# pwrliang/grpc-rdma

Hardware: AMD Instinct MI355X
Metric: streaming GiB/s @1 MiB msgs (client-streaming, 1 connection per GPU) (higher is better)
Workload: dtype u8

## Files before the change

grpc-rdma_amd/csrc/grdma_dev.h:

```cpp
#ifndef GRDMA_DEV_H
#define GRDMA_DEV_H

#include <stddef.h>
#include <stdint.h>

#define GRDMA_ALIGN 8ull
#define GRDMA_RESERVED 24ull
#define GRDMA_FOOTER 0xFFFFFFFFFFFFFFFFull

#define GRDMA_MAX_SEGS 16384
#define GRDMA_MAX_SLICES 8192
#define GRDMA_TX_MAX_RECORDS 4096
#define GRDMA_HINT_MAX_RECORDS 8192
#define GRDMA_RX_HIST 1024
#define GRDMA_RX_TAB_SLOTS 8u
#define GRDMA_RX_TAB_STRIDE 516u
#define GRDMA_RX_TAB_WORDS (4u + 6u * GRDMA_RX_TAB_STRIDE)
#define GRDMA_RX_TAB_MAGIC 0x7AB1E5u
#define GRDMA_RX_HIST_ALLOC_WORDS (GRDMA_RX_HIST + GRDMA_RX_TAB_SLOTS * GRDMA_RX_TAB_WORDS)
#define GRDMA_TILE_BYTES 8192ull
#define GRDMA_PLAN_TILE_SHIFT(ring_cap) ((ring_cap) >= (32ull << 20) ? 14u : 13u)
#define GRDMA_MIN_READ_SLICE 256ull

#ifndef GRDMA_PAIR_STATUS_DEFINED
// ... 127 lines not shown
  uint64_t consumed;
  uint64_t records;
  uint64_t would_block;
  uint64_t credit_sent;
  uint64_t credit_head;
  uint64_t head, moving_head, remain;
  uint64_t arena_used;
  uint64_t zero_off[2];
  uint64_t zero_len[2];
  uint64_t seq;
  uint64_t commit_seq;
  uint32_t pad1;
  uint32_t pad0;
  uint64_t dbg[16];
};

struct grdma_plan {
  uint32_t nsegs;
  uint32_t ntiles;
  uint64_t bytes;
  uint64_t tag_base;
  uint64_t tag_mask;
  uint32_t tile_bytes;
  uint32_t ready;
  struct grdma_seg segs[GRDMA_MAX_SEGS];
  uint32_t tile_prefix[GRDMA_MAX_SEGS + 1];
  uint32_t pad_line0[31];
  uint32_t blocks_done;
  uint32_t mw_arrive;
  uint32_t promise_done;
  uint32_t pad_p;
  uint64_t promise;
  uint32_t mw_done;
  uint32_t pad_line1[25];
};
static_assert(offsetof(grdma_plan, promise) % 8 == 0, "the hand-over word is a 64-bit atomic");

#define GRDMA_JOB_HOOK_ARGS 10
struct grdma_job_hook {
  const void* fn;
  uint32_t grid, threads;
  uint64_t args[GRDMA_JOB_HOOK_ARGS];
};

#endif
```

grpc-rdma_amd/csrc/grdma_rx_fast.h:

```cpp
#ifndef GRDMA_RX_FAST_H
#define GRDMA_RX_FAST_H
#include "grdma_dev.h"
#include "grdma_devfn.h"
#include "grdma_ops.h"

namespace {

#define RXF_THREADS 1024
#define RXF_PER 4
#define RXF_KERNEL_ATTR
#define RXF_MAX (RXF_THREADS * RXF_PER)
#define RXF_WAVES (RXF_THREADS / 64)
#define RXF_MINRD 256u
#define RXF_PMAX 512u
#define RXF_LOOKBACK 192u

__device__ unsigned long long g_rx_fast_drains[6] = {0, 0, 0, 0, 0, 0};

#define RXG_BULK 4096
#define RXG_PAD(i) ((i) + ((i) >> 4))
struct rx_lds_general {
  uint32_t hist[GRDMA_RX_HIST];
  uint32_t penc[RXG_PAD(RXG_BULK) + 1];
  uint32_t xenc[RXG_PAD(RXG_BULK + 1) + 1];
// ... 78 lines not shown
__device__ __forceinline__ rxf_layout rxf_lay(uint32_t n, uint32_t s_in, uint32_t pay, uint32_t cap, uint32_t cap_open,
                                              bool odd, uint32_t ts) {
  rxf_layout L;
  const rxf_rec rp = rxf_replay(n, s_in);
  L.sl0 = (rp.sl0 == RXF_MINRD && s_in != 0) ? cap_open : rp.sl0;
  L.sl1 = rp.sl1;
  L.sl_cnt = rp.sl_cnt;
  L.bytes = rxf_al16(L.sl0) + rxf_al16(L.sl1);
  const uint32_t filled = s_in ? cap_open - s_in : 0;
  const uint32_t d2 = (odd && rp.c2) ? rxf_al16(cap_open) : filled + rp.c1;
  const uint32_t mask = cap - 1;
  const uint32_t p0 = pay, l_a = rp.c1 < cap - p0 ? rp.c1 : cap - p0;
  const uint32_t p2 = (pay + rp.c1) & mask, l_c = rp.c2 < cap - p2 ? rp.c2 : cap - p2;
  L.off[0] = p0;  L.len[0] = l_a;          L.dst_rel[0] = filled;
  L.off[1] = 0;   L.len[1] = rp.c1 - l_a;  L.dst_rel[1] = filled + l_a;
  L.off[2] = p2;  L.len[2] = l_c;          L.dst_rel[2] = d2;
  L.off[3] = 0;   L.len[3] = rp.c2 - l_c;  L.dst_rel[3] = d2 + l_c;
  if (pay + n <= cap && L.len[2] != 0 && d2 == filled + rp.c1) {
    L.len[0] += L.len[2];
    L.len[2] = 0;
  }
  L.nsg = 0;
  L.ntl = 0;
#pragma unroll
  for (int k = 0; k < 4; k++) {
    L.nsg += L.len[k] ? 1u : 0u;
    L.ntl += rxf_tiles(L.len[k], ts);
  }
  return L;
}

struct rxf_counters {
  uint64_t total_read, credit_msgs, rx_records, rx_rounds, seq;
  uint32_t h1;
  grdma_hostline* line;
};
__device__ __forceinline__ rxf_counters rxf_load_counters(const grdma_conn* c, const grdma_rx_result* res) {
  return {c->total_read, c->credit_msgs, c->rx_records, c->rx_rounds, res->seq, c->rx_h1, c->line};
}

template <class Tail>
__device__ __forceinline__ void rxf_commit(const grdma_rx_op& op, bool cursors, uint8_t* ring, uint64_t cap64, uint64_t head64, uint64_t mh0,
                                           uint64_t irs0, uint32_t Lr, uint32_t ts,
                                           uint32_t V, uint32_t tot_n, uint32_t tot_sl, uint32_t tot_sg, uint32_t tot_tl, uint32_t tot_by,
                                           uint32_t short_len, uint32_t leftover_final,
                                           uint64_t slice_idx0, uint64_t a_off0, uint64_t a_end, uint64_t hc, const Tail& tail,
                                           bool crossed, uint64_t base, uint64_t credit, uint64_t credit_head, const rxf_counters& o,
                                           uint64_t t_begin, uint64_t t_pattern, uint64_t t_probe, uint64_t t_state, uint64_t t_scan,
                                           uint64_t t_emit, uint32_t P, uint32_t nwg, uint64_t d_arrived, uint64_t d_loaded,
                                           uint64_t d_credit) {
  grdma_conn* const c = op.conn;
  grdma_plan* const plan = op.plan;
  grdma_rx_result* const res = op.result;
  grdma_slice_out* const out_slices = op.slices + slice_idx0;
  const uint32_t nsl_final = tot_sl + (short_len ? 1u : 0u);
  const uint64_t Ctot = Lr;
  const uint64_t irs = crossed ? Ctot - base : irs0 + Ctot;
  const uint64_t nh = (head64 + Lr) & (cap64 - 1);
  if (short_len) {
    out_slices[tot_sl].off = a_off0 + tot_by;
    out_slices[tot_sl].len = short_len;
  }
  plan->nsegs = tot_sg;
  plan->ntiles = tot_tl;
  plan->tile_bytes = 1u << ts;
  plan->tile_prefix[tot_sg] = tot_tl;
  plan->bytes = tot_n;
  plan->tag_base = (uint64_t)ring;
  plan->tag_mask = cap64 - 1;
  plan->blocks_done = 0;
  c->head = nh;
// ... 27 lines not shown
  res->consumed = Lr;
  res->records = V;
  res->would_block = 1;
  res->credit_sent = credit;
  res->head = nh;
  res->moving_head = nh;
  res->remain = 0;
  res->arena_used = a_end;
  res->zero_off[0] = res->zero_off[1] = res->zero_len[0] = res->zero_len[1] = 0;
  if (nh > mh0) {
    res->zero_off[0] = mh0;
    res->zero_len[0] = nh - mh0;
  } else {
    res->zero_off[0] = mh0;
    res->zero_len[0] = cap64 - mh0;
    res->zero_off[1] = 0;
    res->zero_len[1] = nh;
  }
  res->dbg[0] = t_begin;
  res->dbg[2] = t_pattern - t_begin;
  res->dbg[3] = t_probe - t_begin;
  res->dbg[4] = t_state - t_begin;
  res->dbg[5] = t_scan - t_begin;
  res->dbg[6] = t_emit - t_begin;
  res->dbg[7] = V;
  res->dbg[8] = P;
  res->dbg[9] = 0xFA57;
  if (nwg) {
    res->dbg[10] = nwg;
    res->dbg[11] = d_arrived;
    res->dbg[12] = d_loaded;
    res->dbg[13] = d_credit;
  }
  res->pad1++;
  res->dbg[1] = __builtin_amdgcn_s_memtime();
  atomicAdd(&g_rx_fast_drains[0], 1ull);
  __hip_atomic_store(&res->seq, op.seq_next ? op.seq_next : o.seq + 1, __ATOMIC_RELAXED, __HIP_MEMORY_SCOPE_SYSTEM);
}

__device__ __forceinline__ void rxf_scan3(uint32_t v0, uint32_t v1, uint32_t v2, uint32_t (*s_w)[RXF_WAVES],
                                          uint32_t* x0, uint32_t* x1, uint32_t* x2, uint32_t tot[3]) {
  const int lane = threadIdx.x & 63, wave = threadIdx.x >> 6;
  const uint32_t i0 = wave_incl_scan_u32(v0), i1 = wave_incl_scan_u32(v1), i2 = wave_incl_scan_u32(v2);
  if (lane == 63) {
    s_w[0][wave] = i0;
    s_w[1][wave] = i1;
    s_w[2][wave] = i2;
  }
  __syncthreads();
  uint32_t b0 = 0, b1 = 0, b2 = 0, t0 = 0, t1 = 0, t2 = 0;
#pragma unroll
  for (int w = 0; w < RXF_WAVES; w++) {
    const uint32_t a = s_w[0][w], b = s_w[1][w], c = s_w[2][w];
    if (w < wave) { b0 += a; b1 += b; b2 += c; }
    t0 += a; t1 += b; t2 += c;
  }
  __syncthreads();
  *x0 = b0 + i0 - v0;
  *x1 = b1 + i1 - v1;
  *x2 = b2 + i2 - v2;
  tot[0] = t0; tot[1] = t1; tot[2] = t2;
}

#define RXFP(i) ((i) + ((i) / RXF_PER))

__device__ __forceinline__ bool rxf_body(const grdma_rx_op& op_in) {
  const grdma_rx_op op = op_in;
// ... 327 lines not shown
```

grpc-rdma_amd/csrc/grdma_rx_hint.h:

```cpp
#ifndef GRDMA_RX_HINT_H
#define GRDMA_RX_HINT_H
#include <type_traits>
#include "grdma_rx_multi.h"

namespace {

#define RXH_HALF (RXM_G * RXM_THREADS)
#define RXH_MAX (2 * RXH_HALF)
static_assert(RXH_MAX <= GRDMA_HINT_MAX_RECORDS, "the size table of a round covers a drain");

struct rx_lds_hint {
  uint32_t n[RXH_MAX];
  uint32_t x[RXH_MAX + 1];
};

struct rxh_pre {
  uint32_t nv[RXH_HALF / RXM_THREADS];
  uint32_t V;
  uint64_t h_start;
};
__device__ __forceinline__ void rxh_preload(const grdma_rx_op& op, rxh_pre& p) {
  constexpr uint32_t PER = RXH_HALF / RXM_THREADS;
  const grdma_size_hint* const hint = op.sizes_in;
  p.V = 0;
  p.h_start = ~0ull;
#pragma unroll
  for (uint32_t r = 0; r < PER; r++) p.nv[r] = 0;
  if (hint != nullptr) {
    p.h_start = hint->start_off;
    p.V = hint->count;
#pragma unroll
    for (uint32_t r = 0; r < PER; r++) p.nv[r] = hint->n[threadIdx.x * PER + r];
  }
}

template <bool EWT = false, class RingWait = ring_ready_now, class Publish = credit_unpublished>
__device__ __forceinline__ int rxh_body(const grdma_rx_op& op_in, const uint32_t wg, const uint32_t nwg, const rxh_pre* pre = nullptr,
                                        RingWait* ring_wait = nullptr, Publish* publish = nullptr) {
  static_assert(sizeof(rx_lds_hint) <= sizeof(rx_lds), "the tables fit the planners' LDS");
  rx_lds_hint& H = *reinterpret_cast<rx_lds_hint*>(rx_lds_get());
  const grdma_rx_op op = op_in;
  const uint64_t t_begin = __builtin_amdgcn_s_memtime();
  const uint32_t tid = threadIdx.x;
  grdma_conn* c = op.conn;
  grdma_plan* plan = op.plan;
  grdma_rx_result* res = op.result;
  __shared__ uint32_t s_w[4][RXM_WAVES];
  __shared__ uint32_t s_bad, s_bad_ring, s_first, s_F;

  uint8_t* const ring = c->ring;
  const uint64_t cap64 = c->cap;
  const uint64_t head64 = c->head, mh0 = c->moving_head, remain0 = c->remain, leftover0 = c->leftover_cap;
  const uint64_t irs0 = c->internal_read_size;
  const uint64_t hc = c->rx_hist_count;
  const uint32_t status = c->status;
  const uint64_t lim = op.limit_ptr ? __hip_atomic_load(op.limit_ptr, __ATOMIC_RELAXED, __HIP_MEMORY_SCOPE_AGENT) : 0;
  const uint64_t slice_idx0 = op.append == 1 ? c->rx_slice_idx : 0;
  const uint64_t a_off0 = op.append == 1 ? c->rx_arena_off : 0;
  const grdma_size_hint* const hint = op.sizes_in;
  const uint64_t h_start = pre ? pre->h_start : (hint ? hint->start_off : ~0ull);
  const uint32_t V = pre ? pre->V : (hint ? hint->count : 0);

  const bool search_due = V > RXH_HALF && c->rx_period == 0 && hc >= c->rx_period_retry_at;
  bool ok = !search_due && status == GRDMA_PAIR_CONNECTED && op.raw_cap == 0 && op.append != 0 && !op.inline_apply &&
            op.limit_ptr != nullptr && remain0 == 0 && leftover0 <= RXF_MINRD && cap64 <= (1ull << 31) &&
            a_off0 < (1ull << 31) && hint != nullptr && h_start == head64 && V != 0 && V <= nwg * RXM_CHUNK && V <= RXH_MAX;
  uint64_t max_slices = GRDMA_MAX_SLICES;
  {
    const uint64_t room = op.slices_cap > slice_idx0 ? op.slices_cap - slice_idx0 : 0;
    if (room < max_slices) max_slices = room;
    if (op.max_reads < max_slices) max_slices = op.max_reads;
  }
  const uint32_t cap = (uint32_t)cap64, mask = cap - 1u, head = (uint32_t)head64;
  const uint32_t Lr = ((uint32_t)lim - head) & mask;
  const bool idle = Lr == 0;
  if (tid == 0) {
    s_bad = 0;
    s_bad_ring = 0;
    s_first = RXM_NONE;
    s_F = RXM_NONE;
  }
  __syncthreads();
  uint32_t reason = (!ok || idle) ? 1u : 0u;
  const uint32_t ts = GRDMA_PLAN_TILE_SHIFT(cap64);

  constexpr uint32_t PER = RXH_HALF / RXM_THREADS;
  if (!reason) {
    bool bad = false;
    uint32_t base_x = 0;
    auto load_half = [&](auto HALF) {
      constexpr uint32_t half = decltype(HALF)::value;
      uint32_t nv[PER];
      const uint32_t i0 = half * RXH_HALF + tid * PER;
#pragma unroll
      for (uint32_t r = 0; r < PER; r++)
        nv[r] = (half == 0 && pre) ? pre->nv[r] : hint->n[i0 + r < V ? i0 + r : 0];
      uint32_t sum = 0;
#pragma unroll
      for (uint32_t r = 0; r < PER; r++) {
        if (i0 + r >= V) nv[r] = 0;
        else bad |= nv[r] == 0 || nv[r] > cap - (uint32_t)GRDMA_RESERVED;
        sum += i0 + r < V ? 16u + ((nv[r] + 7u) & ~7u) : 0u;
      }
      uint32_t px, d1, d2, d3, tot[4];
      rxm_scan4(sum, 0, 0, 0, s_w, &px, &d1, &d2, &d3, tot);
      px += base_x;
#pragma unroll
      for (uint32_t r = 0; r < PER; r++) {
        H.n[i0 + r] = nv[r];
        H.x[i0 + r] = px;
        px += i0 + r < V ? 16u + ((nv[r] + 7u) & ~7u) : 0u;
      }
      if (tid == RXM_THREADS - 1) H.x[(half + 1) * RXH_HALF] = px;
      base_x += tot[0];
    };
    load_half(std::integral_constant<uint32_t, 0>{});
    if (V > RXH_HALF) load_half(std::integral_constant<uint32_t, 1>{});
    if (bad) s_bad = 1;
    __syncthreads();
    if (s_bad || H.x[V] != Lr) reason = 2;
  }
  const uint64_t t_pattern = __builtin_amdgcn_s_memtime();
  if (ring_wait != nullptr) (*ring_wait)();

  const uint32_t i_mine = wg * RXM_CHUNK + tid;
  const bool have = !reason && i_mine < V;
  uint32_t xe = 0, n_mine = 0;
  if (!reason) {
    typedef uint32_t u32x2 __attribute__((ext_vector_type(2)));
    const uint32_t ring_lo = (uint32_t)__builtin_amdgcn_readfirstlane((int)(uint32_t)(uint64_t)ring);
    const uint32_t ring_hi = (uint32_t)__builtin_amdgcn_readfirstlane((int)(uint32_t)((uint64_t)ring >> 32));
    const uint64_t ring_u = ((uint64_t)ring_hi << 32) | (uint64_t)ring_lo;
    const uint32_t cap_u = (uint32_t)__builtin_amdgcn_readfirstlane((int)cap);
    const __amdgpu_buffer_rsrc_t rs = __builtin_amdgcn_make_buffer_rsrc((void*)ring_u, 0, cap_u, 0x00020000);
    uint32_t ee = 0;
    if (have) {
      xe = H.x[i_mine];
      n_mine = H.n[i_mine];
      ee = 16u + ((n_mine + 7u) & ~7u);
    }
    const uint32_t o_h = have ? ((head + xe) & mask & ~7u) : 0u;
    const uint32_t o_f = have ? ((head + xe + ee - 8u) & mask & ~7u) : 0u;
    const u32x2 hw = __builtin_amdgcn_raw_buffer_load_b64(rs, o_h, 0, 16 );
    const u32x2 fw = __builtin_amdgcn_raw_buffer_load_b64(rs, o_f, 0, 16);
    if (have) {
      const uint64_t h = ((uint64_t)hw.y << 32) | hw.x, f = ((uint64_t)fw.y << 32) | fw.x;
      if (h != (uint64_t)n_mine || f != GRDMA_FOOTER) s_bad_ring = 1;
// ... 62 lines not shown
      m_by = Lm.bytes;
    }
    if (far) s_bad = 1;
    uint32_t d0, d1, d2, d3, ta[4], tz[4], tm[4];
    rxm_scan4(a_pk, a_tl, a_by, a_n, s_w, &d0, &d1, &d2, &d3, ta);
    rxm_scan4(z_pk, z_tl, z_by, z_n, s_w, &d0, &d1, &d2, &d3, tz);
    rxm_scan4(m_pk, m_tl, m_by, have ? n_mine : 0u, s_w, &x_pk, &x_tl, &x_by, &d3, tm);
    b_pk = ta[0]; b_tl = ta[1]; b_by = ta[2];
    tot_pk = ta[0] + tm[0] + tz[0];
    tot_tl = ta[1] + tm[1] + tz[1];
    tot_by = ta[2] + tm[2] + tz[2];
    tot_n = ta[3] + tm[3] + tz[3];
    if (s_bad) reason = 4;
    if (!reason) {
      bool far2 = false;
      s_end = rxf_space_after(H.n[V - 1], state_of(V - 1, &far2));
    }
  }
  const uint64_t t_state = __builtin_amdgcn_s_memtime();
  const uint32_t tot_sl = tot_pk & 0xFFFFu, tot_sg = tot_pk >> 16;
  const uint32_t cap_open_end = (odd_open && first_done == RXM_NONE) ? s0 : RXF_MINRD;
  const uint32_t short_len = s_end ? cap_open_end - s_end : 0;
  const uint32_t nsl_final = tot_sl + (short_len ? 1u : 0u);
  const uint32_t leftover_final = s_end ? s_end : RXF_MINRD;
  const uint64_t a_end = a_off0 + tot_by + rxf_al16(short_len);
  if (!reason && !(nsl_final + 2 <= max_slices && tot_sg + 8 <= GRDMA_MAX_SEGS && a_end + leftover_final + 16 <= op.arena_cap &&
                   a_end < (1ull << 32)))
    reason = 5;
  const uint64_t t_scan = __builtin_amdgcn_s_memtime();
  const bool committer = wg == nwg - 1;
  GRDMA_WAIT_LOADS();
  __syncthreads();
  if (tid == 0) drain_count_in(plan, reason);

  grdma_slice_out* const out_slices = op.slices + slice_idx0;
  if (!reason && have) {
    const uint32_t pk = b_pk + x_pk;
    uint32_t sl = pk & 0xFFFFu, sg = pk >> 16, tl = b_tl + x_tl;
    const uint64_t A = a_off0 + b_by + x_by;
    int last_piece = 0;
#pragma unroll
    for (int k = 1; k < 4; k++)
      if (Lm.len[k]) last_piece = k;
#pragma unroll
    for (int k = 0; k < 4; k++) {
      if (Lm.len[k] == 0) continue;
      const uint64_t fl = GRDMA_SEG_ZERO_SRC | (k == 0 ? GRDMA_SEG_TAG_HDR : 0) | (k == last_piece ? GRDMA_SEG_TAG_FTR : 0);
      xwg_put_seg<EWT>(&plan->segs[sg], (uint64_t)op.arena + A + Lm.dst_rel[k], (uint64_t)(ring + Lm.off[k]), (uint64_t)Lm.len[k], fl);
      xwg_st32<EWT>(&plan->tile_prefix[sg], tl);
      sg++;
      tl += rxf_tiles(Lm.len[k], ts);
    }
    uint64_t sof = A;
    if (Lm.sl0) {
      xwg_st64<EWT>(&out_slices[sl].off, sof);
      xwg_st64<EWT>(&out_slices[sl].len, (uint64_t)Lm.sl0);
      sl++;
      sof += rxf_al16(Lm.sl0);
    }
    if (Lm.sl1) {
      xwg_st64<EWT>(&out_slices[sl].off, sof);
      xwg_st64<EWT>(&out_slices[sl].len, (uint64_t)Lm.sl1);
    }
  }
  rxf_counters o = {};
  uint64_t base = 0, credit = 0, credit_head = 0;
  bool crossed = false;
  if (tid == 0 && !reason && committer) {
    o = rxf_load_counters(c, res);
    const uint64_t T = cap64 / 2, Ctot = Lr;
    uint64_t thr = T - irs0;
    while (Ctot >= thr) {
      uint32_t lo = 0, hi = V - 1;
      const uint32_t t32 = (uint32_t)thr;
      while (lo < hi) {
        const uint32_t mid = (lo + hi) >> 1;
        if (H.x[mid + 1] >= t32) hi = mid; else lo = mid + 1;
      }
      const uint32_t n = H.n[lo];
      bool far = false;
      rxf_credit_step(n, rxf_replay(n, state_of(lo, &far)), (uint64_t)H.x[lo + 1], head64, cap64, T, thr, base, credit, credit_head, crossed);
    }
  }
  const uint64_t t_emit = __builtin_amdgcn_s_memtime();

  if (!committer) {
    if (EWT) GRDMA_WAIT_VMEM();
    __syncthreads();
    if (tid == 0) drain_leave(plan);
    return 0;
  }
  const uint32_t s_any = drain_verdicts(plan, nwg);
  if (s_any) {
    if (tid == 0) {
      atomicAdd(&g_rx_fast_drains[reason ? reason : 3u], 1ull);
      atomicAdd(&g_rx_verdicts[s_any < nwg ? 0 : 1], 1ull);
      if (!idle) res->pad0++;
    }
    if (EWT) GRDMA_WAIT_VMEM();
    if (tid == 0) drain_close(plan, nwg);
    __syncthreads();
    return 2;
  }
  if (tid == 0 && publish != nullptr) (*publish)(credit, credit_head);

  constexpr int NH = GRDMA_RX_HIST / RXM_THREADS;
#pragma unroll
  for (int r = 0; r < NH; r++) {
    const uint32_t back = tid + r * RXM_THREADS;
    if (back < V) {
      const uint32_t i = V - 1 - back;
      c->rx_hist[(uint32_t)((hc + i) % GRDMA_RX_HIST)] = 16u + ((H.n[i] + 7u) & ~7u);
    }
  }
  if (tid == 0) {
    auto tail = [&](uint32_t& h1, uint32_t& h2) {
      h1 = 16u + ((H.n[V - 1] + 7u) & ~7u);
      h2 = V >= 2 ? 16u + ((H.n[V - 2] + 7u) & ~7u) : o.h1;
    };
    rxf_commit(op, true , ring, cap64, head64, mh0, irs0, Lr, ts,
               V, tot_n, tot_sl, tot_sg, tot_tl, tot_by, short_len, leftover_final,
               slice_idx0, a_off0, a_end, hc, tail,
               crossed, base, credit, credit_head, o,
               t_begin, t_pattern, t_probe, t_state, t_scan, t_emit, 0 , nwg, 0, 0, 0);
    drain_close(plan, nwg);
  }
  return 1;
}

}
#endif
```

grpc-rdma_amd/csrc/grdma_rx_multi.h:

```cpp
#ifndef GRDMA_RX_MULTI_H
#define GRDMA_RX_MULTI_H
#include "grdma_rx_fast.h"

namespace {

#define RXM_THREADS 256u
#define RXM_WAVES (RXM_THREADS / 64u)
#define RXM_G 16u
#define RXM_CHUNK RXM_THREADS
#define RXM_PFX (RXF_LOOKBACK + 1u)
#define RXM_RESET (2u * RXF_MINRD)
#define RXM_NONE 0xFFFFFFFFu

__device__ unsigned long long g_rx_tab_stats[2] = {0, 0};
__device__ unsigned long long g_rx_verdicts[2] = {0, 0};

struct rx_lds_multi {
  uint32_t hist[GRDMA_RX_HIST];
  uint32_t pat[RXF_PMAX], pre[RXF_PMAX + 1];
  uint32_t npat[RXF_PMAX];
  uint16_t sss[RXF_PMAX];
  uint32_t qpk[RXF_PMAX + 1], qtl[RXF_PMAX + 1], qby[RXF_PMAX + 1];
  uint32_t qn[RXF_PMAX + 1];
  uint16_t as[RXM_PFX + 1];
  uint32_t apk[RXM_PFX + 1], atl[RXM_PFX + 1], aby[RXM_PFX + 1];
};

__device__ __forceinline__ void rxm_scan4(uint32_t v0, uint32_t v1, uint32_t v2, uint32_t v3, uint32_t (*s_w)[RXM_WAVES],
                                          uint32_t* x0, uint32_t* x1, uint32_t* x2, uint32_t* x3, uint32_t tot[4]) {
  const int lane = threadIdx.x & 63, wave = threadIdx.x >> 6;
  const uint32_t i0 = wave_incl_scan_u32(v0), i1 = wave_incl_scan_u32(v1), i2 = wave_incl_scan_u32(v2), i3 = wave_incl_scan_u32(v3);
  if (lane == 63) {
    s_w[0][wave] = i0;
    s_w[1][wave] = i1;
    s_w[2][wave] = i2;
    s_w[3][wave] = i3;
  }
  __syncthreads();
  uint32_t b0 = 0, b1 = 0, b2 = 0, b3 = 0, t0 = 0, t1 = 0, t2 = 0, t3 = 0;
#pragma unroll
  for (int w = 0; w < (int)RXM_WAVES; w++) {
    const uint32_t a = s_w[0][w], b = s_w[1][w], c = s_w[2][w], d = s_w[3][w];
    if (w < wave) { b0 += a; b1 += b; b2 += c; b3 += d; }
    t0 += a; t1 += b; t2 += c; t3 += d;
  }
  __syncthreads();
  *x0 = b0 + i0 - v0;
  *x1 = b1 + i1 - v1;
  *x2 = b2 + i2 - v2;
  *x3 = b3 + i3 - v3;
  tot[0] = t0; tot[1] = t1; tot[2] = t2; tot[3] = t3;
}

__device__ __forceinline__ uint32_t rxm_div(uint32_t k, uint32_t P, uint32_t inv) { return P > 1 ? (uint32_t)(((uint64_t)k * inv) >> 32) : k; }

__device__ __forceinline__ void rxm_cyc(const rx_lds_multi& M, uint32_t P, uint32_t inv, uint32_t k, uint32_t* pk, uint32_t* tl, uint32_t* by) {
  const uint32_t q = rxm_div(k, P, inv), r = k - q * P;
  *pk = q * M.qpk[P] + M.qpk[r];
  *tl = q * M.qtl[P] + M.qtl[r];
  *by = q * M.qby[P] + M.qby[r];
}

__device__ unsigned long long g_wire_wait_runout = 0;
__device__ __forceinline__ void wire_arrive(grdma_plan* wp) {
  __builtin_amdgcn_fence(__ATOMIC_RELEASE, "agent");
  __hip_atomic_fetch_add(&wp->mw_arrive, 1u, __ATOMIC_RELAXED, __HIP_MEMORY_SCOPE_AGENT);
}
__device__ __forceinline__ void wire_wait(grdma_plan* wp, uint32_t wire_groups, uint32_t participants) {
  if (threadIdx.x == 0) {
    bool seen = false;
    for (uint32_t spins = 0; spins < (1u << 22) && !seen; spins++) {
      seen = __hip_atomic_load(&wp->mw_arrive, __ATOMIC_RELAXED, __HIP_MEMORY_SCOPE_AGENT) >= wire_groups;
      if (!seen) __builtin_amdgcn_s_sleep(2);
    }
    if (!seen) atomicAdd(&g_wire_wait_runout, 1ull);
    const uint32_t prev = __hip_atomic_fetch_add(&wp->promise_done, 1u, __ATOMIC_RELAXED, __HIP_MEMORY_SCOPE_AGENT);
    if (prev + 1 == participants) {
      __hip_atomic_store(&wp->promise_done, 0u, __ATOMIC_RELAXED, __HIP_MEMORY_SCOPE_AGENT);
      __hip_atomic_store(&wp->mw_arrive, 0u, __ATOMIC_RELAXED, __HIP_MEMORY_SCOPE_AGENT);
    }
  }
  __syncthreads();
}
struct ring_ready_now {
  __device__ __forceinline__ void operator()() {}
};
struct ring_behind_wire {
  grdma_plan* wp;
  uint32_t wire_groups, participants;
  bool done;
  __device__ __forceinline__ void operator()() {
    if (wp != nullptr && !done) wire_wait(wp, wire_groups, participants);
    done = true;
  }
};
struct credit_unpublished {
  __device__ __forceinline__ void operator()(uint64_t, uint64_t) {}
};
struct credit_promised {
  grdma_plan* plan;
  uint32_t participants;
  bool done;
  __device__ __forceinline__ void operator()(uint64_t credit_sent, uint64_t credit_head) {
    if (plan != nullptr && !done) (void)promise_keep(plan, participants, credit_sent, credit_head);
    done = true;
  }
};

__device__ __forceinline__ void drain_count_in(grdma_plan* plan, uint32_t reason) {
  __hip_atomic_fetch_add(&plan->mw_arrive, 1u + (reason ? 0x10000u : 0u), __ATOMIC_RELAXED, __HIP_MEMORY_SCOPE_AGENT);
}
__device__ __forceinline__ void drain_leave(grdma_plan* plan) {
  __hip_atomic_fetch_add(&plan->mw_done, 1u, __ATOMIC_RELAXED, __HIP_MEMORY_SCOPE_AGENT);
}
__device__ __forceinline__ uint32_t drain_verdicts(grdma_plan* plan, uint32_t nwg) {
  __shared__ uint32_t s_declined;
  if (threadIdx.x == 0) {
    uint32_t v = 0;
    for (uint32_t spins = 0; spins < (1u << 22); spins++) {
      v = __hip_atomic_load(&plan->mw_arrive, __ATOMIC_RELAXED, __HIP_MEMORY_SCOPE_AGENT);
      if ((v & 0xFFFFu) >= nwg) break;
      __builtin_amdgcn_s_sleep(1);
    }
    s_declined = (v & 0xFFFFu) >= nwg ? (v >> 16) : nwg;
  }
  __syncthreads();
  return s_declined;
}
__device__ __forceinline__ void drain_close(grdma_plan* plan, uint32_t nwg) {
  for (uint32_t spins = 0; spins < (1u << 22); spins++) {
    if (__hip_atomic_load(&plan->mw_done, __ATOMIC_RELAXED, __HIP_MEMORY_SCOPE_AGENT) >= nwg - 1) break;
    __builtin_amdgcn_s_sleep(1);
  }
  __hip_atomic_store(&plan->mw_done, 0u, __ATOMIC_RELAXED, __HIP_MEMORY_SCOPE_AGENT);
  __hip_atomic_store(&plan->mw_arrive, 0u, __ATOMIC_RELAXED, __HIP_MEMORY_SCOPE_AGENT);
}

template <bool EWT = false, class RingWait = ring_ready_now, class Publish = credit_unpublished>
__device__ __forceinline__ int rxm_body(const grdma_rx_op& op_in, const uint32_t wg, const uint32_t nwg, RingWait* ring_wait = nullptr,
                                        Publish* publish = nullptr) {
  static_assert(sizeof(rx_lds_multi) <= sizeof(rx_lds), "the tables fit their LDS");
  rx_lds_multi& M = *reinterpret_cast<rx_lds_multi*>(rx_lds_get());
  const grdma_rx_op op = op_in;
  const uint64_t t_begin = __builtin_amdgcn_s_memtime();
  const uint32_t tid = threadIdx.x;
  grdma_conn* c = op.conn;
  grdma_plan* plan = op.plan;
  grdma_rx_result* res = op.result;
  __shared__ uint32_t s_w[4][RXM_WAVES];
  __shared__ uint32_t s_bad, s_vj, s_first, s_F, s_miss, s_lb;

  uint8_t* const ring = c->ring;
  const uint64_t cap64 = c->cap;
  const uint64_t head64 = c->head, mh0 = c->moving_head, remain0 = c->remain, leftover0 = c->leftover_cap;
  const uint64_t irs0 = c->internal_read_size;
  const uint64_t hc = c->rx_hist_count;
  const uint32_t P = c->rx_period;
  const uint32_t status = c->status;
  const uint32_t* const gh = c->rx_hist;
  const bool limited = op.limit_ptr != nullptr || c->wire_limit != 0;
  const uint64_t lim = op.limit_ptr ? __hip_atomic_load(op.limit_ptr, __ATOMIC_RELAXED, __HIP_MEMORY_SCOPE_AGENT)
                                    : __hip_atomic_load(&c->wire_recv.wire_tail, __ATOMIC_RELAXED, __HIP_MEMORY_SCOPE_SYSTEM);
  const uint64_t slice_idx0 = op.append == 1 ? c->rx_slice_idx : 0;
  const uint64_t a_off0 = op.append == 1 ? c->rx_arena_off : 0;
  constexpr int NH = GRDMA_RX_HIST / RXM_THREADS;
  uint32_t hv[NH];
#pragma unroll
  for (int r = 0; r < NH; r++) hv[r] = gh[tid + r * RXM_THREADS];
// ... 3 lines not shown
            cap64 <= (1ull << 31) && a_off0 < (1ull << 31);
  uint64_t max_slices = GRDMA_MAX_SLICES;
  {
    const uint64_t room = op.slices_cap > slice_idx0 ? op.slices_cap - slice_idx0 : 0;
    if (room < max_slices) max_slices = room;
    if (op.max_reads < max_slices) max_slices = op.max_reads;
  }
  const uint32_t cap = (uint32_t)cap64, mask = cap - 1u, head = (uint32_t)head64;
  const uint32_t Lr = ((uint32_t)lim - head) & mask;
  const bool idle = Lr == 0;
  const uint32_t invP = P > 1 ? (uint32_t)(0xFFFFFFFFu / P) + 1u : 0u;
  auto divP = [&](uint32_t k) -> uint32_t { return rxm_div(k, P, invP); };
  if (tid == 0) {
    s_bad = 0;
    s_vj = RXM_NONE;
    s_first = RXM_NONE;
    s_F = RXM_NONE;
    s_miss = 0;
    s_lb = 0;
  }
  uint32_t c_hdr[4] = {0, 0, 0, 0}, c_key[2] = {0, 0}, c_sss[2] = {0, 0}, c_qpk[2] = {0, 0}, c_qtl[2] = {0, 0}, c_qby[2] = {0, 0},
           c_qn[2] = {0, 0}, c_tot[4] = {0, 0, 0, 0};
  uint32_t* c_tab = nullptr;
#pragma unroll
  for (int r = 0; r < NH; r++) M.hist[tid + r * RXM_THREADS] = hv[r];
  __syncthreads();
  uint32_t reason = (!ok || idle) ? 1u : 0u;

  uint32_t SP = 0, V = 0;
  if (!reason) {
    const uint32_t j0 = 2 * tid, j1 = j0 + 1;
    const uint32_t pv0 = j0 < P ? M.hist[(uint32_t)((hc - P + j0) % GRDMA_RX_HIST)] : 0;
    const uint32_t pv1 = j1 < P ? M.hist[(uint32_t)((hc - P + j1) % GRDMA_RX_HIST)] : 0;
    uint32_t px, d1, d2, d3, ptot[4];
    rxm_scan4(pv0 + pv1, 0, 0, 0, s_w, &px, &d1, &d2, &d3, ptot);
    SP = ptot[0];
    if (j0 < P) {
      M.pat[j0] = pv0;
      M.pre[j0] = px;
    }
    if (j1 < P) {
      M.pat[j1] = pv1;
      M.pre[j1] = px + pv0;
    }
    if (tid == 0) M.pre[P] = SP;
    const uint32_t q_full = SP ? Lr / SP : 0, rem = SP ? Lr - q_full * SP : 0;
    if (SP != 0) {
      if (j0 < P && px == rem) s_vj = j0;
      if (j1 < P && px + pv0 == rem) s_vj = j1;
    }
    __syncthreads();
    const uint32_t vj = s_vj;
    const uint64_t V64 = (uint64_t)q_full * P + vj;
    if (SP == 0 || vj == RXM_NONE || V64 == 0 || V64 > (uint64_t)nwg * RXM_CHUNK) reason = 2;
    else V = (uint32_t)V64;
  }
  const uint32_t ts = GRDMA_PLAN_TILE_SHIFT(cap64);
  const uint64_t t_pattern = __builtin_amdgcn_s_memtime();
  if (reason && !idle && op.sizes_in != nullptr) return 3;
  if (ring_wait != nullptr) (*ring_wait)();

  const uint32_t i_mine = wg * RXM_CHUNK + tid;
  const bool have = !reason && i_mine < V;
  const uint32_t PV = reason ? 0u : (V < P ? V : P);
  uint32_t xe = 0, ee = 0, ri_mine = 0, n_mine = 0;
  if (!reason) {
    typedef uint32_t u32x2 __attribute__((ext_vector_type(2)));
    const uint32_t ring_lo = (uint32_t)__builtin_amdgcn_readfirstlane((int)(uint32_t)(uint64_t)ring);
    const uint32_t ring_hi = (uint32_t)__builtin_amdgcn_readfirstlane((int)(uint32_t)((uint64_t)ring >> 32));
// ... 232 lines not shown
      while (hi - lo > 1) {
        const uint32_t mid = (lo + hi) >> 1;
        if (M.pre[mid] <= r) lo = mid; else hi = mid;
      }
      const uint32_t w = q * P + lo;
      if (w >= NF && w < V) {
        const uint32_t n = M.npat[lo], s = M.sss[lo];
        const rxf_layout La = rxf_lay(n, s, (head + q * SP + M.pre[lo] + 8u) & mask, cap, RXF_MINRD, false, ts);
        w_rec = w;
        d_sg = La.nsg - ((M.qpk[lo + 1] - M.qpk[lo]) >> 16);
        d_tl = La.ntl - (M.qtl[lo + 1] - M.qtl[lo]);
      }
    }
    if (V > NF) before(V, &tot_pk, &tot_tl, &tot_by);
    else { tot_pk = PS_pk; tot_tl = PS_tl; tot_by = PS_by; }
    uint32_t n_last;
    const uint32_t s_last_in = state_of(V - 1, &n_last);
    s_end = rxf_space_after(n_last, s_last_in);
  }
  const uint32_t tot_sl = tot_pk & 0xFFFFu, tot_sg = tot_pk >> 16;
  const uint32_t cap_open_end = (odd_open && first_done == RXM_NONE) ? s0 : RXF_MINRD;
  const uint32_t short_len = s_end ? cap_open_end - s_end : 0;
  const uint32_t nsl_final = tot_sl + (short_len ? 1u : 0u);
  const uint32_t leftover_final = s_end ? s_end : RXF_MINRD;
  const uint64_t a_end = a_off0 + tot_by + rxf_al16(short_len);
  if (!reason && !(nsl_final + 2 <= max_slices && tot_sg + 8 <= GRDMA_MAX_SEGS && a_end + leftover_final + 16 <= op.arena_cap &&
                   a_end < (1ull << 32)))
    reason = 5;
  const uint64_t t_scan = __builtin_amdgcn_s_memtime();
  const bool committer = wg == nwg - 1;
  GRDMA_WAIT_LOADS();
  __syncthreads();
  if (tid == 0) drain_count_in(plan, reason);

  grdma_slice_out* const out_slices = op.slices + slice_idx0;
  if (!reason && have) {
    uint32_t n, pk, tl, by;
    const uint32_t s_in = state_of(i_mine, &n);
    if (i_mine < NF) {
      pk = M.apk[i_mine];
      tl = M.atl[i_mine];
      by = M.aby[i_mine];
    } else {
      before(i_mine, &pk, &tl, &by);
    }
    uint32_t sl = pk & 0xFFFFu, sg = pk >> 16;
    const bool in_first = odd_open && i_mine <= first_done;
    const rxf_layout L = rxf_lay(n, s_in, (head + xe + 8u) & mask, cap, in_first ? s0 : RXF_MINRD,
                                 odd_open && i_mine == first_done, ts);
    const uint64_t A = a_off0 + by;
    int last_piece = 0;
#pragma unroll
    for (int k = 1; k < 4; k++)
      if (L.len[k]) last_piece = k;
#pragma unroll
    for (int k = 0; k < 4; k++) {
      if (L.len[k] == 0) continue;
      const uint64_t fl = GRDMA_SEG_ZERO_SRC | (k == 0 ? GRDMA_SEG_TAG_HDR : 0) | (k == last_piece ? GRDMA_SEG_TAG_FTR : 0);
      xwg_put_seg<EWT>(&plan->segs[sg], (uint64_t)op.arena + A + L.dst_rel[k], (uint64_t)(ring + L.off[k]), (uint64_t)L.len[k], fl);
      xwg_st32<EWT>(&plan->tile_prefix[sg], tl);
      sg++;
      tl += rxf_tiles(L.len[k], ts);
    }
    uint64_t sof = A;
    if (L.sl0) {
      xwg_st64<EWT>(&out_slices[sl].off, sof);
      xwg_st64<EWT>(&out_slices[sl].len, (uint64_t)L.sl0);
      sl++;
      sof += rxf_al16(L.sl0);
// ... 12 lines not shown
      const uint32_t qi = divP(i), ri = i - qi * P;
      return (uint64_t)qi * SP + M.pre[ri] + M.pat[ri];
    };
    const uint64_t T = cap64 / 2, Ctot = Lr;
    uint64_t thr = T - irs0;
    while (Ctot >= thr) {
      uint32_t lo;
      {
        const uint32_t t32 = (uint32_t)thr;
        const uint32_t qk = t32 / SP, r = t32 - qk * SP;
        uint32_t a = 0, b = P;
        if (r == 0) b = 0;
        while (b - a > 1) {
          const uint32_t mid = (a + b) >> 1;
          if (M.pre[mid] >= r) b = mid; else a = mid;
        }
        const uint32_t k = qk * P + b;
        lo = k ? k - 1 : 0;
        if (lo > V - 1) lo = V - 1;
      }
      uint32_t n;
      const uint32_t s_in = state_of(lo, &n);
      rxf_credit_step(n, rxf_replay(n, s_in), enc_end(lo), head64, cap64, T, thr, base, credit, credit_head, crossed);
    }
  }
  const uint64_t t_emit = __builtin_amdgcn_s_memtime();

  if (!committer) {
    if (EWT) GRDMA_WAIT_VMEM();
    __syncthreads();
    if (tid == 0) drain_leave(plan);
    return 0;
  }
  const uint32_t s_any = drain_verdicts(plan, nwg);
  if (c_fresh) {
    uint32_t* const a = c_tab + 4;
#pragma unroll
    for (int r = 0; r < 2; r++) {
      const uint32_t pj = 2 * tid + r;
      if (pj < P) {
        a[pj] = M.npat[pj];
        a[GRDMA_RX_TAB_STRIDE + pj] = (uint32_t)M.sss[pj];
        a[2 * GRDMA_RX_TAB_STRIDE + pj] = M.qpk[pj];
        a[3 * GRDMA_RX_TAB_STRIDE + pj] = M.qtl[pj];
        a[4 * GRDMA_RX_TAB_STRIDE + pj] = M.qby[pj];
        a[5 * GRDMA_RX_TAB_STRIDE + pj] = M.qn[pj];
      }
    }
    if (tid == 0) {
      a[2 * GRDMA_RX_TAB_STRIDE + RXF_PMAX] = M.qpk[P];
      a[3 * GRDMA_RX_TAB_STRIDE + RXF_PMAX] = M.qtl[P];
      a[4 * GRDMA_RX_TAB_STRIDE + RXF_PMAX] = M.qby[P];
      a[5 * GRDMA_RX_TAB_STRIDE + RXF_PMAX] = M.qn[P];
      c_tab[0] = P;
      c_tab[1] = ts;
      c_tab[2] = s_lb;
      c_tab[3] = GRDMA_RX_TAB_MAGIC;
    }
  }
  const uint64_t t_arrived = __builtin_amdgcn_s_memtime();
  if (s_any) {
    if (tid == 0) {
      atomicAdd(&g_rx_fast_drains[reason ? reason : 3u], 1ull);
      atomicAdd(&g_rx_verdicts[s_any < nwg ? 0 : 1], 1ull);
      if (!idle) res->pad0++;
    }
    if (EWT) GRDMA_WAIT_VMEM();
    if (tid == 0) drain_close(plan, nwg);
    __syncthreads();
    return 2;
  }
  if (tid == 0 && publish != nullptr) (*publish)(credit, credit_head);

  if (tid == 0) atomicAdd(&g_rx_tab_stats[c_hit ? 0 : 1], 1ull);
#pragma unroll
  for (int r = 0; r < NH; r++) {
    const uint32_t back = tid + r * RXM_THREADS;
    if (back < V) {
      const uint32_t i = V - 1 - back;
      c->rx_hist[(uint32_t)((hc + i) % GRDMA_RX_HIST)] = M.pat[i - divP(i) * P];
    }
  }
  if (tid == 0) {
    const uint64_t t_loaded = __builtin_amdgcn_s_memtime() + (o.seq & 0);
    const uint32_t tot_n = divP(V) * M.qn[P] + M.qn[V - divP(V) * P];
    const uint64_t t_credit = __builtin_amdgcn_s_memtime();
    auto tail = [&](uint32_t& h1, uint32_t& h2) {
      const uint32_t rl = (V - 1) - divP(V - 1) * P;
      h1 = M.pat[rl];
      h2 = V >= 2 ? M.pat[rl ? rl - 1 : P - 1] : o.h1;
    };
    rxf_commit(op, op.append != 0, ring, cap64, head64, mh0, irs0, Lr, ts,
               V, tot_n, tot_sl, tot_sg, tot_tl, tot_by, short_len, leftover_final,
               slice_idx0, a_off0, a_end, hc, tail,
               crossed, base, credit, credit_head, o,
               t_begin, t_pattern, t_probe, t_state, t_scan, t_emit, P, nwg, t_arrived - t_begin,
               t_loaded - t_begin, t_credit - t_begin);
    drain_close(plan, nwg);
  }
  return 1;
}

}
#endif
```

Measured before the change: 680.4.

## Use epoch-based drain counters and hoist history tail fetch before verdict wait

```diff
diff --git a/grpc-rdma_amd/csrc/grdma_dev.h b/grpc-rdma_amd/csrc/grdma_dev.h
--- a/grpc-rdma_amd/csrc/grdma_dev.h
+++ b/grpc-rdma_amd/csrc/grdma_dev.h
@@ -183,9 +183,14 @@
   uint32_t pad_p;
   uint64_t promise;
   uint32_t mw_done;
-  uint32_t pad_line1[25];
+  uint32_t mw_done_base;
+  uint64_t mw_count;
+  uint64_t mw_count_base;
+  uint32_t mw_resync;
+  uint32_t pad_line1[19];
 };
 static_assert(offsetof(grdma_plan, promise) % 8 == 0, "the hand-over word is a 64-bit atomic");
+static_assert(offsetof(grdma_plan, mw_count) % 8 == 0, "the count-in word is a 64-bit atomic");
 
 #define GRDMA_JOB_HOOK_ARGS 10
 struct grdma_job_hook {
diff --git a/grpc-rdma_amd/csrc/grdma_rx_fast.h b/grpc-rdma_amd/csrc/grdma_rx_fast.h
--- a/grpc-rdma_amd/csrc/grdma_rx_fast.h
+++ b/grpc-rdma_amd/csrc/grdma_rx_fast.h
@@ -134,11 +134,11 @@
 
 struct rxf_counters {
   uint64_t total_read, credit_msgs, rx_records, rx_rounds, seq;
-  uint32_t h1;
+  uint32_t h1, taken;
   grdma_hostline* line;
 };
 __device__ __forceinline__ rxf_counters rxf_load_counters(const grdma_conn* c, const grdma_rx_result* res) {
-  return {c->total_read, c->credit_msgs, c->rx_records, c->rx_rounds, res->seq, c->rx_h1, c->line};
+  return {c->total_read, c->credit_msgs, c->rx_records, c->rx_rounds, res->seq, c->rx_h1, res->pad1, c->line};
 }
 
 template <class Tail>
@@ -232,7 +232,7 @@
     res->dbg[12] = d_loaded;
     res->dbg[13] = d_credit;
   }
-  res->pad1++;
+  res->pad1 = o.taken + 1;
   res->dbg[1] = __builtin_amdgcn_s_memtime();
   atomicAdd(&g_rx_fast_drains[0], 1ull);
   __hip_atomic_store(&res->seq, op.seq_next ? op.seq_next : o.seq + 1, __ATOMIC_RELAXED, __HIP_MEMORY_SCOPE_SYSTEM);
diff --git a/grpc-rdma_amd/csrc/grdma_rx_hint.h b/grpc-rdma_amd/csrc/grdma_rx_hint.h
--- a/grpc-rdma_amd/csrc/grdma_rx_hint.h
+++ b/grpc-rdma_amd/csrc/grdma_rx_hint.h
@@ -53,6 +53,7 @@
   const uint64_t head64 = c->head, mh0 = c->moving_head, remain0 = c->remain, leftover0 = c->leftover_cap;
   const uint64_t irs0 = c->internal_read_size;
   const uint64_t hc = c->rx_hist_count;
+  uint32_t* const gh = c->rx_hist;
   const uint32_t status = c->status;
   const uint64_t lim = op.limit_ptr ? __hip_atomic_load(op.limit_ptr, __ATOMIC_RELAXED, __HIP_MEMORY_SCOPE_AGENT) : 0;
   const uint64_t slice_idx0 = op.append == 1 ? c->rx_slice_idx : 0;
@@ -102,8 +103,8 @@
         else bad |= nv[r] == 0 || nv[r] > cap - (uint32_t)GRDMA_RESERVED;
         sum += i0 + r < V ? 16u + ((nv[r] + 7u) & ~7u) : 0u;
       }
-      uint32_t px, d1, d2, d3, tot[4];
-      rxm_scan4(sum, 0, 0, 0, s_w, &px, &d1, &d2, &d3, tot);
+      uint32_t px, tot_x;
+      rxm_scan1(sum, s_w, &px, &tot_x);
       px += base_x;
 #pragma unroll
       for (uint32_t r = 0; r < PER; r++) {
@@ -112,7 +113,7 @@
         px += i0 + r < V ? 16u + ((nv[r] + 7u) & ~7u) : 0u;
       }
       if (tid == RXM_THREADS - 1) H.x[(half + 1) * RXH_HALF] = px;
-      base_x += tot[0];
+      base_x += tot_x;
     };
     load_half(std::integral_constant<uint32_t, 0>{});
     if (V > RXH_HALF) load_half(std::integral_constant<uint32_t, 1>{});
@@ -241,6 +242,8 @@
   GRDMA_WAIT_LOADS();
   __syncthreads();
   if (tid == 0) drain_count_in(plan, reason);
+  drain_epoch epoch = {};
+  if (tid == 0 && committer) epoch = drain_begin(plan);
 
   grdma_slice_out* const out_slices = op.slices + slice_idx0;
   if (!reason && have) {
@@ -299,7 +302,29 @@
     if (tid == 0) drain_leave(plan);
     return 0;
   }
-  const uint32_t s_any = drain_verdicts(plan, nwg);
+  constexpr int NH = GRDMA_RX_HIST / RXM_THREADS;
+  uint32_t hist_at[NH], hist_val[NH];
+  uint32_t tail_h1 = 0, tail_h2 = 0;
+  auto fetch_tail = [&]() {
+#pragma unroll
+    for (int r = 0; r < NH; r++) {
+      const uint32_t back = tid + r * RXM_THREADS;
+      hist_at[r] = RXM_NONE;
+      hist_val[r] = 0;
+      if (!reason && back < V) {
+        const uint32_t i = V - 1 - back;
+        hist_at[r] = (uint32_t)((hc + i) % GRDMA_RX_HIST);
+        hist_val[r] = 16u + ((H.n[i] + 7u) & ~7u);
+      }
+    }
+    if (tid == 0 && !reason) {
+      tail_h1 = 16u + ((H.n[V - 1] + 7u) & ~7u);
+      tail_h2 = V >= 2 ? 16u + ((H.n[V - 2] + 7u) & ~7u) : o.h1;
+    }
+  };
+  const bool tail_early = publish == nullptr || !publish->pending();
+  if (tail_early) fetch_tail();
+  const uint32_t s_any = drain_verdicts(plan, nwg, epoch);
   if (s_any) {
     if (tid == 0) {
       atomicAdd(&g_rx_fast_drains[reason ? reason : 3u], 1ull);
@@ -307,32 +332,30 @@
       if (!idle) res->pad0++;
     }
     if (EWT) GRDMA_WAIT_VMEM();
-    if (tid == 0) drain_close(plan, nwg);
+    if (tid == 0) {
+      drain_wait_left(plan, nwg, epoch);
+      drain_close(plan, nwg, epoch);
+    }
     __syncthreads();
     return 2;
   }
   if (tid == 0 && publish != nullptr) (*publish)(credit, credit_head);
-
-  constexpr int NH = GRDMA_RX_HIST / RXM_THREADS;
-#pragma unroll
-  for (int r = 0; r < NH; r++) {
-    const uint32_t back = tid + r * RXM_THREADS;
-    if (back < V) {
-      const uint32_t i = V - 1 - back;
-      c->rx_hist[(uint32_t)((hc + i) % GRDMA_RX_HIST)] = 16u + ((H.n[i] + 7u) & ~7u);
-    }
-  }
+  if (!tail_early) fetch_tail();
+
+#pragma unroll
+  for (int r = 0; r < NH; r++)
+    if (hist_at[r] != RXM_NONE) gh[hist_at[r]] = hist_val[r];
   if (tid == 0) {
     auto tail = [&](uint32_t& h1, uint32_t& h2) {
-      h1 = 16u + ((H.n[V - 1] + 7u) & ~7u);
-      h2 = V >= 2 ? 16u + ((H.n[V - 2] + 7u) & ~7u) : o.h1;
+      h1 = tail_h1;
+      h2 = tail_h2;
     };
     rxf_commit(op, true , ring, cap64, head64, mh0, irs0, Lr, ts,
                V, tot_n, tot_sl, tot_sg, tot_tl, tot_by, short_len, leftover_final,
                slice_idx0, a_off0, a_end, hc, tail,
                crossed, base, credit, credit_head, o,
                t_begin, t_pattern, t_probe, t_state, t_scan, t_emit, 0 , nwg, 0, 0, 0);
-    drain_close(plan, nwg);
+    drain_close(plan, nwg, epoch);
   }
   return 1;
 }
diff --git a/grpc-rdma_amd/csrc/grdma_rx_multi.h b/grpc-rdma_amd/csrc/grdma_rx_multi.h
--- a/grpc-rdma_amd/csrc/grdma_rx_multi.h
+++ b/grpc-rdma_amd/csrc/grdma_rx_multi.h
@@ -52,6 +52,23 @@
   tot[0] = t0; tot[1] = t1; tot[2] = t2; tot[3] = t3;
 }
 
+__device__ __forceinline__ void rxm_scan1(uint32_t v0, uint32_t (*s_w)[RXM_WAVES], uint32_t* x0, uint32_t* tot) {
+  const int lane = threadIdx.x & 63, wave = threadIdx.x >> 6;
+  const uint32_t i0 = wave_incl_scan_u32(v0);
+  if (lane == 63) s_w[0][wave] = i0;
+  __syncthreads();
+  uint32_t b0 = 0, t0 = 0;
+#pragma unroll
+  for (int w = 0; w < (int)RXM_WAVES; w++) {
+    const uint32_t a = s_w[0][w];
+    if (w < wave) b0 += a;
+    t0 += a;
+  }
+  __syncthreads();
+  *x0 = b0 + i0 - v0;
+  *tot = t0;
+}
+
 __device__ __forceinline__ uint32_t rxm_div(uint32_t k, uint32_t P, uint32_t inv) { return P > 1 ? (uint32_t)(((uint64_t)k * inv) >> 32) : k; }
 
 __device__ __forceinline__ void rxm_cyc(const rx_lds_multi& M, uint32_t P, uint32_t inv, uint32_t k, uint32_t* pk, uint32_t* tl, uint32_t* by) {
@@ -96,6 +113,7 @@
 };
 struct credit_unpublished {
   __device__ __forceinline__ void operator()(uint64_t, uint64_t) {}
+  __device__ __forceinline__ bool pending() const { return false; }
 };
 struct credit_promised {
   grdma_plan* plan;
@@ -105,35 +123,52 @@
     if (plan != nullptr && !done) (void)promise_keep(plan, participants, credit_sent, credit_head);
     done = true;
   }
+  __device__ __forceinline__ bool pending() const { return plan != nullptr && !done; }
 };
 
+struct drain_epoch {
+  uint64_t count_base;
+  uint32_t done_base, resync;
+};
+__device__ __forceinline__ drain_epoch drain_begin(const grdma_plan* plan) {
+  return {plan->mw_count_base, plan->mw_done_base, plan->mw_resync};
+}
 __device__ __forceinline__ void drain_count_in(grdma_plan* plan, uint32_t reason) {
-  __hip_atomic_fetch_add(&plan->mw_arrive, 1u + (reason ? 0x10000u : 0u), __ATOMIC_RELAXED, __HIP_MEMORY_SCOPE_AGENT);
+  __hip_atomic_fetch_add(&plan->mw_count, 1ull + (reason ? 1ull << 32 : 0ull), __ATOMIC_RELAXED, __HIP_MEMORY_SCOPE_AGENT);
 }
 __device__ __forceinline__ void drain_leave(grdma_plan* plan) {
   __hip_atomic_fetch_add(&plan->mw_done, 1u, __ATOMIC_RELAXED, __HIP_MEMORY_SCOPE_AGENT);
 }
-__device__ __forceinline__ uint32_t drain_verdicts(grdma_plan* plan, uint32_t nwg) {
+__device__ __forceinline__ uint32_t drain_verdicts(grdma_plan* plan, uint32_t nwg, drain_epoch& e) {
   __shared__ uint32_t s_declined;
   if (threadIdx.x == 0) {
-    uint32_t v = 0;
+    const uint32_t lo0 = (uint32_t)e.count_base, hi0 = (uint32_t)(e.count_base >> 32);
+    uint64_t v = 0;
+    bool all = false;
     for (uint32_t spins = 0; spins < (1u << 22); spins++) {
-      v = __hip_atomic_load(&plan->mw_arrive, __ATOMIC_RELAXED, __HIP_MEMORY_SCOPE_AGENT);
-      if ((v & 0xFFFFu) >= nwg) break;
+      v = __hip_atomic_load(&plan->mw_count, __ATOMIC_RELAXED, __HIP_MEMORY_SCOPE_AGENT);
+      all = (uint32_t)v - lo0 >= nwg;
+      if (all) break;
       __builtin_amdgcn_s_sleep(1);
     }
-    s_declined = (v & 0xFFFFu) >= nwg ? (v >> 16) : nwg;
+    const uint32_t declined = (uint32_t)(v >> 32) - hi0 - ((uint32_t)v < lo0 ? 1u : 0u);
+    s_declined = (all && !e.resync) ? declined : nwg;
+    e.count_base = all ? v : (uint64_t)(lo0 + nwg);
+    e.resync = all ? 0u : 1u;
   }
   __syncthreads();
   return s_declined;
 }
-__device__ __forceinline__ void drain_close(grdma_plan* plan, uint32_t nwg) {
+__device__ __forceinline__ void drain_wait_left(grdma_plan* plan, uint32_t nwg, const drain_epoch& e) {
   for (uint32_t spins = 0; spins < (1u << 22); spins++) {
-    if (__hip_atomic_load(&plan->mw_done, __ATOMIC_RELAXED, __HIP_MEMORY_SCOPE_AGENT) >= nwg - 1) break;
+    if (__hip_atomic_load(&plan->mw_done, __ATOMIC_RELAXED, __HIP_MEMORY_SCOPE_AGENT) - e.done_base >= nwg - 1) break;
     __builtin_amdgcn_s_sleep(1);
   }
-  __hip_atomic_store(&plan->mw_done, 0u, __ATOMIC_RELAXED, __HIP_MEMORY_SCOPE_AGENT);
-  __hip_atomic_store(&plan->mw_arrive, 0u, __ATOMIC_RELAXED, __HIP_MEMORY_SCOPE_AGENT);
+}
+__device__ __forceinline__ void drain_close(grdma_plan* plan, uint32_t nwg, const drain_epoch& e) {
+  plan->mw_count_base = e.count_base;
+  plan->mw_done_base = e.done_base + (nwg - 1);
+  plan->mw_resync = e.resync;
 }
 
 template <bool EWT = false, class RingWait = ring_ready_now, class Publish = credit_unpublished>
@@ -203,9 +238,8 @@
     const uint32_t j0 = 2 * tid, j1 = j0 + 1;
     const uint32_t pv0 = j0 < P ? M.hist[(uint32_t)((hc - P + j0) % GRDMA_RX_HIST)] : 0;
     const uint32_t pv1 = j1 < P ? M.hist[(uint32_t)((hc - P + j1) % GRDMA_RX_HIST)] : 0;
-    uint32_t px, d1, d2, d3, ptot[4];
-    rxm_scan4(pv0 + pv1, 0, 0, 0, s_w, &px, &d1, &d2, &d3, ptot);
-    SP = ptot[0];
+    uint32_t px;
+    rxm_scan1(pv0 + pv1, s_w, &px, &SP);
     if (j0 < P) {
       M.pat[j0] = pv0;
       M.pre[j0] = px;
@@ -504,9 +538,36 @@
   GRDMA_WAIT_LOADS();
   __syncthreads();
   if (tid == 0) drain_count_in(plan, reason);
+  drain_epoch epoch = {};
+  if (tid == 0 && committer) epoch = drain_begin(plan);
 
   grdma_slice_out* const out_slices = op.slices + slice_idx0;
-  if (!reason && have) {
+  const bool plain = have && i_mine >= NF && i_mine != w_rec && !(odd_open && i_mine <= first_done);
+  if (!reason && __ballot(have && !plain) == 0) {
+    if (have) {
+      uint32_t n, pk, tl, by;
+      const uint32_t s_in = state_of(i_mine, &n);
+      before(i_mine, &pk, &tl, &by);
+      uint32_t sl = pk & 0xFFFFu;
+      const uint32_t sg = pk >> 16;
+      const rxf_rec rp = rxf_replay(n, s_in);
+      const uint64_t A = a_off0 + by;
+      xwg_put_seg<EWT>(&plan->segs[sg], (uint64_t)op.arena + A + (s_in ? RXF_MINRD - s_in : 0u), (uint64_t)(ring + ((head + xe + 8u) & mask)),
+                       (uint64_t)n, GRDMA_SEG_ZERO_SRC | GRDMA_SEG_TAG_HDR | GRDMA_SEG_TAG_FTR);
+      xwg_st32<EWT>(&plan->tile_prefix[sg], tl);
+      uint64_t sof = A;
+      if (rp.sl0) {
+        xwg_st64<EWT>(&out_slices[sl].off, sof);
+        xwg_st64<EWT>(&out_slices[sl].len, (uint64_t)rp.sl0);
+        sl++;
+        sof += rxf_al16(rp.sl0);
+      }
+      if (rp.sl1) {
+        xwg_st64<EWT>(&out_slices[sl].off, sof);
+        xwg_st64<EWT>(&out_slices[sl].len, (uint64_t)rp.sl1);
+      }
+    }
+  } else if (!reason && have) {
     uint32_t n, pk, tl, by;
     const uint32_t s_in = state_of(i_mine, &n);
     if (i_mine < NF) {
@@ -585,7 +646,30 @@
     if (tid == 0) drain_leave(plan);
     return 0;
   }
-  const uint32_t s_any = drain_verdicts(plan, nwg);
+  uint32_t hist_at[NH], hist_val[NH];
+  uint32_t tot_n = 0, tail_h1 = 0, tail_h2 = 0;
+  auto fetch_tail = [&]() {
+#pragma unroll
+    for (int r = 0; r < NH; r++) {
+      const uint32_t back = tid + r * RXM_THREADS;
+      hist_at[r] = RXM_NONE;
+      hist_val[r] = 0;
+      if (!reason && back < V) {
+        const uint32_t i = V - 1 - back;
+        hist_at[r] = (uint32_t)((hc + i) % GRDMA_RX_HIST);
+        hist_val[r] = M.pat[i - divP(i) * P];
+      }
+    }
+    if (tid == 0 && !reason) {
+      tot_n = divP(V) * M.qn[P] + M.qn[V - divP(V) * P];
+      const uint32_t rl = (V - 1) - divP(V - 1) * P;
+      tail_h1 = M.pat[rl];
+      tail_h2 = V >= 2 ? M.pat[rl ? rl - 1 : P - 1] : o.h1;
+    }
+  };
+  const bool tail_early = publish == nullptr || !publish->pending();
+  if (tail_early) fetch_tail();
+  const uint32_t s_any = drain_verdicts(plan, nwg, epoch);
   if (c_fresh) {
     uint32_t* const a = c_tab + 4;
 #pragma unroll
@@ -619,29 +703,27 @@
       if (!idle) res->pad0++;
     }
     if (EWT) GRDMA_WAIT_VMEM();
-    if (tid == 0) drain_close(plan, nwg);
+    if (tid == 0) {
+      drain_wait_left(plan, nwg, epoch);
+      drain_close(plan, nwg, epoch);
+    }
     __syncthreads();
     return 2;
   }
   if (tid == 0 && publish != nullptr) (*publish)(credit, credit_head);
+  if (!tail_early) fetch_tail();
 
   if (tid == 0) atomicAdd(&g_rx_tab_stats[c_hit ? 0 : 1], 1ull);
-#pragma unroll
-  for (int r = 0; r < NH; r++) {
-    const uint32_t back = tid + r * RXM_THREADS;
-    if (back < V) {
-      const uint32_t i = V - 1 - back;
-      c->rx_hist[(uint32_t)((hc + i) % GRDMA_RX_HIST)] = M.pat[i - divP(i) * P];
-    }
-  }
+  uint32_t* const hist_out = const_cast<uint32_t*>(gh);
+#pragma unroll
+  for (int r = 0; r < NH; r++)
+    if (hist_at[r] != RXM_NONE) hist_out[hist_at[r]] = hist_val[r];
   if (tid == 0) {
     const uint64_t t_loaded = __builtin_amdgcn_s_memtime() + (o.seq & 0);
-    const uint32_t tot_n = divP(V) * M.qn[P] + M.qn[V - divP(V) * P];
-    const uint64_t t_credit = __builtin_amdgcn_s_memtime();
+    const uint64_t t_credit = t_loaded;
     auto tail = [&](uint32_t& h1, uint32_t& h2) {
-      const uint32_t rl = (V - 1) - divP(V - 1) * P;
-      h1 = M.pat[rl];
-      h2 = V >= 2 ? M.pat[rl ? rl - 1 : P - 1] : o.h1;
+      h1 = tail_h1;
+      h2 = tail_h2;
     };
     rxf_commit(op, op.append != 0, ring, cap64, head64, mh0, irs0, Lr, ts,
                V, tot_n, tot_sl, tot_sg, tot_tl, tot_by, short_len, leftover_final,
@@ -649,7 +731,7 @@
                crossed, base, credit, credit_head, o,
                t_begin, t_pattern, t_probe, t_state, t_scan, t_emit, P, nwg, t_arrived - t_begin,
                t_loaded - t_begin, t_credit - t_begin);
-    drain_close(plan, nwg);
+    drain_close(plan, nwg, epoch);
   }
   return 1;
 }
```

Measured after the change: 684.6, median of 6. About the same (+0.6%).
